# lmcinnes/pynndescent

Hardware: AMD Instinct MI355X
Metric: index build: points indexed/sec (recall@10 vs brute force reported alongside) (higher is better)
Workload: dtype f32

## Files before the change

include/pynnd_amd.h:

```cpp
#ifndef PYNND_AMD_H
#define PYNND_AMD_H

#include <stdint.h>

#ifdef __cplusplus
extern "C" {
#endif

#define NND_METRIC_SQEUCLIDEAN 0
#define NND_METRIC_ALT_COSINE 1

#define NND_ABI_VERSION 6

typedef struct nnd_handle_s *nnd_handle_t;

typedef struct nnd_params {
    int64_t n;
    int32_t dim;
    int32_t metric;
    int32_t n_neighbors;
    int32_t n_trees;
    int32_t leaf_size;
    int32_t max_depth;
    int32_t max_candidates;
// ... 11 lines not shown
#define NND_FLAG_NO_PREP 2
#define NND_FLAG_TEST_SELECT_WAVE 4
#define NND_FLAG_TEST_SMALL_REGIONS 8
#define NND_FLAG_TEST_ROUTE_PLAIN 16
#define NND_FLAG_TEST_FOREST_BY_TREE 32
#define NND_FLAG_TEST_FAIL 64
#define NND_FLAG_TEST_VANISH 128
#define NND_FLAG_TEST_SAMPLE_ATOMIC 256
#define NND_FLAG_TEST_FOREST_FALLBACK_TOPS 512
#define NND_FLAG_TEST_FOREST_FALLBACK_SHARE 1024
#define NND_TEST_FALLBACK_AT(flags) ((((flags) & 512) ? 1 : 0) + (((flags) & 1024) ? 2 : 0))
#define NND_FLAG_TEST_SAMPLE_NOMEM 2048
#define NND_FLAG_TEST_SELECT_HALF 4096
#define NND_FLAG_TEST_GATHER_INLINE 8192
#define NND_FLAG_TEST_JOIN_UNSTAGED 16384

typedef struct nnd_stats {
    int64_t n_iters_run;
    int64_t n_leaves;
    int64_t tree_levels;
    int64_t leaf_pairs;
    int64_t leaf_rows;
    int64_t join_pairs[64];
    int64_t join_rows[64];
    int64_t join_active[64];
    int64_t proposals[64];
    int64_t updates[64];
    float ms_prep, ms_forest, ms_leaf_init, ms_random_init, ms_descent, ms_finalize;
    float ms_sample[64], ms_join[64], ms_merge[64];
    int64_t join_mfma[64];
// ... 168 lines not shown
```

pynndescent_amd/_capi.py:

```python
import ctypes as C
import os

import numpy as np

_HERE = os.path.dirname(os.path.abspath(__file__))
LIB_PATH = os.environ.get("PYNND_AMD_LIB", os.path.join(_HERE, "libpynnd_amd.so"))

NND_METRIC_SQEUCLIDEAN = 0
NND_METRIC_ALT_COSINE = 1
METRIC_CODES = {"euclidean": NND_METRIC_SQEUCLIDEAN, "l2": NND_METRIC_SQEUCLIDEAN, "sqeuclidean": NND_METRIC_SQEUCLIDEAN,
                "cosine": NND_METRIC_ALT_COSINE}
NND_FLAG_NO_GRAPH = 1
NND_FLAG_NO_PREP = 2
NND_FLAG_TEST_SELECT_WAVE = 4
NND_FLAG_TEST_SMALL_REGIONS = 8
NND_FLAG_TEST_ROUTE_PLAIN = 16
NND_FLAG_TEST_FOREST_BY_TREE = 32
NND_FLAG_TEST_FAIL = 64
NND_FLAG_TEST_VANISH = 128
NND_FLAG_TEST_FOREST_FALLBACK_TOPS = 512
NND_FLAG_TEST_FOREST_FALLBACK_SHARE = 1024
NND_FLAG_TEST_GATHER_INLINE = 8192
NND_FLAG_TEST_JOIN_UNSTAGED = 16384
NND_FLAG_TEST_SELECT_HALF = 4096
NND_FLAG_TEST_SAMPLE_NOMEM = 2048
NND_FLAG_TEST_SAMPLE_ATOMIC = 256


class NNDParams(C.Structure):
    _fields_ = [
        ("n", C.c_int64),
        ("dim", C.c_int32),
        ("metric", C.c_int32),
        ("n_neighbors", C.c_int32),
        ("n_trees", C.c_int32),
        ("leaf_size", C.c_int32),
        ("max_depth", C.c_int32),
        ("max_candidates", C.c_int32),
        ("n_iters", C.c_int32),
        ("delta", C.c_float),
        ("rng_state", C.c_int64 * 3),
# ... 574 lines not shown
```

pynndescent_amd/csrc/capi.hip:

```cpp
#include <stdlib.h>
#include <string.h>

#include <atomic>
#include <mutex>
#include <string>
#include <thread>
#include <vector>

#include "common.h"
#include "state.h"

static thread_local char g_err[512] = {0};

static void gerr(const char *fmt, ...) {
    va_list ap;
    va_start(ap, fmt);
    vsnprintf(g_err, sizeof(g_err), fmt, ap);
    va_end(ap);
}

extern "C" int32_t nnd_abi_version(void) { return NND_ABI_VERSION; }
extern "C" const char *nnd_last_global_error(void) { return g_err; }
extern "C" const char *nnd_last_error(nnd_handle_t h) { return h ? h->err : g_err; }

// ... 49 lines not shown
#endif
    return m;
}

static void free_all(nnd_ctx *ctx) {
    auto F = [](void *p) {
        if (p) (void)hipFree(p);
    };
    if (ctx->x_owned) F((void *)ctx->x_orig);
    for (void *&a : ctx->slim_alloc) { F(a); a = nullptr; }
    F(ctx->xp); F(ctx->nrm); F(ctx->nr2); F(ctx->xh); F(ctx->mean); F(ctx->knn_e); F(ctx->knn_d); F(ctx->th); F(ctx->pbuf_r);
    F(ctx->pdirty); F(ctx->out_idx); F(ctx->out_dist);
    F(ctx->rv_pos); F(ctx->rv_in_cursor); F(ctx->rv_in_rec); F(ctx->rv_ov);
    for (int i = 0; i < 2; i++) { F(ctx->perm[i]); F(ctx->pos_seg[i]); F(ctx->seg_start[i]); F(ctx->seg_len[i]); }
    F(ctx->inv); F(ctx->side); F(ctx->side_pt); F(ctx->leaf_flag); F(ctx->scan_out); F(ctx->scan_blk); F(ctx->seg_nleft); F(ctx->seg_child);
    F(ctx->xs); F(ctx->xsh); F(ctx->nr2s); F(ctx->node_hf); F(ctx->node_hh); F(ctx->node_child); F(ctx->node_pack); F(ctx->node_hfc); F(ctx->route_roots); F(ctx->route_ws); F(ctx->s_leaf_depth);
    F(ctx->cell_count); F(ctx->cell_start); F(ctx->cell_depth); F(ctx->small_list);
    F(ctx->hyper); F(ctx->hyper_h); F(ctx->leaf_start); F(ctx->leaf_len); F(ctx->wl_start); F(ctx->wl_len); F(ctx->colsum_partial); F(ctx->counters_sum);
    if (ctx->h_pin) { (void)hipHostFree(ctx->h_pin); ctx->h_pin = nullptr; }
    if (ctx->h_tree_begin) { (void)hipHostFree(ctx->h_tree_begin); ctx->h_tree_begin = nullptr; }
    F(ctx->tree_begin_dev); F(ctx->counters);
    if (ctx->ev0) (void)hipEventDestroy(ctx->ev0);
    if (ctx->ev1) (void)hipEventDestroy(ctx->ev1);
    if (ctx->ev_spin) (void)hipEventDestroy(ctx->ev_spin);
    for (hipEvent_t e : ctx->tev) if (e) (void)hipEventDestroy(e);
    ctx->tev.clear();
    F(ctx->shard_bounds); F(ctx->shard_cursors);
    nnd_hub_tree_free(ctx);
    nnd_search_graph_free(ctx);
    if (ctx->stream && ctx->stream_owned) (void)hipStreamDestroy(ctx->stream);
}
// ... 147 lines not shown
                if (ctx->cell_leaf < 8) ctx->cell_leaf = 8;
                const int64_t Ps = (int64_t)p->n_trees * ctx->s_m;
                ctx->node_cap = Ps / (ctx->cell_leaf / 4 > 1 ? ctx->cell_leaf / 4 : 1) + 4 * p->n_trees + 64;
                ctx->cell_cap = ctx->node_cap + p->n_trees;
                ctx->max_segs += ctx->cell_cap;
                if ((rc = dalloc(ctx, &ctx->xs, (size_t)ctx->s_m * ctx->dp))) break;
                if ((rc = dalloc(ctx, &ctx->xsh, (size_t)ctx->s_m * ctx->dp))) break;
                if ((rc = dalloc(ctx, &ctx->nr2s, (size_t)ctx->s_m))) break;
                if ((rc = dalloc(ctx, &ctx->node_hf, (size_t)ctx->node_cap * (ctx->dp + 4)))) break;
                if ((rc = dalloc(ctx, &ctx->node_hh, (size_t)ctx->node_cap * ctx->dp))) break;
                if ((rc = dalloc(ctx, &ctx->node_child, (size_t)ctx->node_cap * 2))) break;
                if ((rc = dalloc(ctx, &ctx->node_pack, (size_t)ctx->node_cap * (2 * ctx->dp + 16)))) break;
                if ((rc = dalloc(ctx, &ctx->node_hfc, (size_t)ctx->node_cap * (ctx->dp + 4)))) break;
                if ((rc = dalloc(ctx, &ctx->route_roots, (size_t)4096))) break;
                if ((rc = dalloc(ctx, &ctx->s_leaf_depth, (size_t)Ps))) break;
                if ((rc = dalloc(ctx, &ctx->cell_count, (size_t)ctx->cell_cap))) break;
                if ((rc = dalloc(ctx, &ctx->cell_start, (size_t)ctx->cell_cap))) break;
                if ((rc = dalloc(ctx, &ctx->cell_depth, (size_t)ctx->cell_cap))) break;
                if ((rc = dalloc(ctx, &ctx->small_list, (size_t)ctx->cell_cap * 3))) break;
            }
            const size_t S = (size_t)ctx->max_segs;
            for (int i = 0; i < 2 && !rc; i++) {
                if ((rc = dalloc(ctx, &ctx->perm[i], P))) break;
                if ((rc = dalloc(ctx, &ctx->pos_seg[i], P))) break;
                if ((rc = dalloc(ctx, &ctx->seg_start[i], S))) break;
                if ((rc = dalloc(ctx, &ctx->seg_len[i], S))) break;
            }
            if (rc) break;
            if ((rc = dalloc(ctx, &ctx->inv, P))) break;
            if ((rc = dalloc(ctx, &ctx->side, P))) break;
// ... 833 lines not shown
```

pynndescent_amd/csrc/rpforest.hip:

```cpp
#include <atomic>
#include <chrono>

#include "common.h"
#include "state.h"

#define RP_EPS 1e-8f

static constexpr int SCAN_ITEMS = 8;
static constexpr int SCAN_BLOCK = 256;
static constexpr int SCAN_TILE = SCAN_ITEMS * SCAN_BLOCK;

__global__ void k_forest_init(int32_t *__restrict__ perm, int32_t *__restrict__ pos_seg, uint8_t *__restrict__ leaf_flag,
                              int32_t *__restrict__ inv, int64_t n, int64_t P, int splittable) {
    int64_t g = (int64_t)blockIdx.x * blockDim.x + threadIdx.x;
    if (g >= P) return;
    int64_t t = g / n;
    int64_t i = g - t * n;
    perm[g] = (int32_t)i;
    inv[g] = splittable ? (int32_t)t : -1;
    pos_seg[g] = splittable ? (int32_t)t : -1;
    leaf_flag[g] = (!splittable && i == 0) ? 1 : 0;
}
__global__ void k_forest_init_segs(int32_t *__restrict__ seg_start, int32_t *__restrict__ seg_len, int n_trees,
                                   int64_t n) {
    int t = blockIdx.x * blockDim.x + threadIdx.x;
    if (t < n_trees) {
        seg_start[t] = (int32_t)(t * n);
        seg_len[t] = (int32_t)n;
    }
}

__global__ __launch_bounds__(256) void k_hyperplane(const float *__restrict__ xp, int dp, const int32_t *__restrict__ perm,
                                                    const int32_t *__restrict__ seg_start,
                                                    const int32_t *__restrict__ seg_len, int n_segs, int angular,
                                                    uint32_t seed, int depth, float *__restrict__ hyper, int hs,
                                                    uint16_t *__restrict__ hyper_h, uint32_t pos_bias, const float *__restrict__ scal) {
    int lane = nnd_lane();
    int s = blockIdx.x * (blockDim.x >> 6) + (threadIdx.x >> 6);
    if (s >= n_segs) return;
    int a = seg_start[s], len = seg_len[s];
    uint32_t li = nnd_hash3(seed, (uint32_t)a + pos_bias, (uint32_t)(2 * depth)) % (uint32_t)len;
    uint32_t ri = nnd_hash3(seed, (uint32_t)a + pos_bias, (uint32_t)(2 * depth + 1)) % (uint32_t)len;
    if (ri == li) ri = (ri + 1) % (uint32_t)len;
    const float *xl = xp + (int64_t)perm[a + li] * dp;
    const float *xr = xp + (int64_t)perm[a + ri] * dp;
    float *h = hyper + (int64_t)s * hs;
    uint16_t *hb = hyper_h + (int64_t)s * dp;
    const float hsc = scal[0], hinv = 1.0f / hsc;
    float acc = 0.0f, sq = 0.0f, res = 0.0f;
    for (int j = lane; j < dp; j += 64) {
        float l = xl[j], r = xr[j];
        float v = l - r;
        h[j] = v;
        if (!angular) {
            const uint16_t b = nnd_f32_to_h16(v, hsc);
            hb[j] = b;
            const float e = v - nnd_h16_to_f32(b, hinv);
            res += e * e;
        }
        acc += angular ? v * v : v * (l + r);
        sq += v * v;
    }
// ... 14 lines not shown
        if (lane == 0) {
            h[dp] = 0.0f;
            h[dp + 1] = nh * inv;
            h[dp + 2] = sqrtf(res) * 1.000001f;
        }
    } else {
        res = nnd_wave_sum_f32(res);
        if (lane == 0) {
            h[dp] = -0.5f * acc;
            h[dp + 1] = sqrtf(sq);
            h[dp + 2] = sqrtf(res) * 1.000001f;
        }
    }
}

#define RP_BAND 0.00786f
#define RP_ACC 3e-5f
#ifdef NND_RP_ALWAYS_EXACT
#define RP_IN_BAND(m, band) ((band) >= 0.0f || (m) == (m))
#else
#define RP_IN_BAND(m, band) (!(fabsf(m) > (band)))
#endif
__device__ __forceinline__ float rp_band(float xnorm, float rx, float hnorm, float rh) {
    return rx * hnorm + (xnorm + rx) * rh + RP_ACC * hnorm * xnorm + RP_EPS;
}
__device__ __forceinline__ uint32_t rp_bf16_up(float v) { return (__float_as_uint(v) + 0xFFFFu) >> 16; }
typedef _Float16 rp_h16x2 __attribute__((ext_vector_type(2)));
__device__ __forceinline__ float rp_dot8(uint4 q, uint4 p, float acc) {
    acc = __builtin_amdgcn_fdot2(__builtin_bit_cast(rp_h16x2, q.x), __builtin_bit_cast(rp_h16x2, p.x), acc, false);
    acc = __builtin_amdgcn_fdot2(__builtin_bit_cast(rp_h16x2, q.y), __builtin_bit_cast(rp_h16x2, p.y), acc, false);
// ... 15 lines not shown
        acc += a.x * b.x + a.y * b.y + a.z * b.z + a.w * b.w;
    }
    return rp_quad_sum(acc);
}
__device__ __forceinline__ uint8_t rp_side(float m, float band, const float *__restrict__ xf_row, const float *h, float off,
                                           int dp, int sub, uint32_t seed, uint32_t key, int depth) {
#ifdef NND_RP_NORECHECK
    if (band < 0.0f) m = rp_exact_quad(xf_row, h, dp, sub) + off;
#else
    if (RP_IN_BAND(m, band)) m = rp_exact_quad(xf_row, h, dp, sub) + off;
#endif
    if (fabsf(m) < RP_EPS) return (uint8_t)(nnd_hash3(seed ^ 0x5bd1e995u, key, (uint32_t)depth) & 1u);
    return m > 0.0f ? 0 : 1;
}

__global__ __launch_bounds__(256) void k_margin(const float *__restrict__ xp, const uint16_t *__restrict__ xh,
                                                const float2 *__restrict__ nr, int metric, int dp,
                                                const int32_t *__restrict__ perm, const int32_t *__restrict__ pos_seg,
                                                int64_t P, const float *__restrict__ hyper, int hs,
                                                const uint16_t *__restrict__ hyper_h, uint32_t seed, int depth,
                                                uint8_t *__restrict__ side, uint32_t pos_bias, const float *__restrict__ scal) {
    const int sub = threadIdx.x & 3;
    const int64_t g = (int64_t)blockIdx.x * (blockDim.x >> 2) + (threadIdx.x >> 2);
    const int s = g < P ? pos_seg[g] : -1;
    if (s < 0) return;
    const int64_t pt = perm[g];
    const uint4 *x8 = (const uint4 *)(xh + pt * dp);
    const uint4 *h8 = (const uint4 *)(hyper_h + (int64_t)s * dp);
    const float *h = hyper + (int64_t)s * hs;
    const float2 nrv = nr[pt];
    const float xn = nrv.x, rx = nrv.y, off = h[dp], hnorm = h[dp + 1], rh = h[dp + 2];
    float acc = 0.0f;
    for (int c = sub; c < (dp >> 3); c += 16) {
        uint4 q[4], p[4];
#pragma unroll
        for (int j = 0; j < 4; j++) {
            const int cc = c + 4 * j < (dp >> 3) ? c + 4 * j : c;
            q[j] = x8[cc];
            p[j] = h8[cc];
        }
#pragma unroll
        for (int j = 0; j < 4; j++)
            if (c + 4 * j < (dp >> 3)) acc = rp_dot8(q[j], p[j], acc);
    }
    const float m = rp_quad_sum(acc) * scal[1] + off;
    const float band = rp_band(metric == 0 ? sqrtf(xn) : xn, rx, hnorm, rh);
    const uint8_t sd = rp_side(m, band, xp + pt * dp, h, off, dp, sub, seed, (uint32_t)g + pos_bias, depth);
    if (sub == 0) side[g] = sd;
}

__global__ __launch_bounds__(256) void k_margin_fused(const float *__restrict__ xp, const uint16_t *__restrict__ xh,
                                                      const float2 *__restrict__ nr, int metric, int dp, int64_t n,
                                                      int n_trees, const int32_t *__restrict__ seg_pt,
                                                      const float *__restrict__ hyper, int hs,
                                                      const uint16_t *__restrict__ hyper_h, uint32_t seed, int depth,
                                                      uint8_t *__restrict__ side_pt, uint32_t pos_bias, const float *__restrict__ scal) {
    const int sub = threadIdx.x & 3;
    const int64_t i = (int64_t)blockIdx.x * (blockDim.x >> 2) + (threadIdx.x >> 2);
    if (i >= n) return;
    const uint4 *x8 = (const uint4 *)(xh + i * dp);
    const float2 nrv = nr[i];
    const float xn = nrv.x, rx = nrv.y;
    const float xnorm = metric == 0 ? sqrtf(xn) : xn;
    const int nch = dp >> 3;
    for (int t0 = 0; t0 < n_trees; t0 += 4) {
        int sg[4];
        float acc[4];
#pragma unroll
        for (int u = 0; u < 4; u++) {
            sg[u] = t0 + u < n_trees ? seg_pt[(int64_t)(t0 + u) * n + i] : -1;
            acc[u] = 0.0f;
        }
        if (sg[0] < 0 && sg[1] < 0 && sg[2] < 0 && sg[3] < 0) continue;
// ... 12 lines not shown
                    if (c + 4 * j < nch) acc[u] = rp_dot8(q[j], p[j], acc[u]);
            }
        }
#pragma unroll
        for (int u = 0; u < 4; u++) {
            if (sg[u] < 0) continue;
            const float *h = hyper + (int64_t)sg[u] * hs;
            const float off = h[dp], hnorm = h[dp + 1], rh = h[dp + 2];
            const float m = rp_quad_sum(acc[u]) * scal[1] + off;
            const float band = rp_band(xnorm, rx, hnorm, rh);
            const int64_t slot = (int64_t)(t0 + u) * n + i;
            const uint8_t sd = rp_side(m, band, xp + i * dp, h, off, dp, sub, seed, (uint32_t)slot + pos_bias, depth);
            if (sub == 0) side_pt[slot] = sd;
        }
    }
}

__device__ __forceinline__ int scan_flag(int mode, const int32_t *pos_seg, const uint8_t *bytes, int64_t g, int64_t P) {
    if (g >= P) return 0;
    if (mode == 0) {
        const int sg = pos_seg[g];
        const uint8_t b = bytes[g];
        return (sg >= 0) & (b == 0);
    }
    return bytes[g] ? 1 : 0;
}

__global__ __launch_bounds__(SCAN_BLOCK) void k_scan_reduce(int mode, const int32_t *__restrict__ pos_seg,
                                                            uint8_t *__restrict__ bytes, int64_t P,
                                                            int32_t *__restrict__ blk, const int32_t *__restrict__ perm,
// ... 243 lines not shown
    }
    if (active_pos) atomicAdd((unsigned long long *)&counters[CNT_LEAVES], (unsigned long long)active_pos);
    if (max_stay) atomicMax((unsigned long long *)&counters[CNT_SCRATCH + 3], (unsigned long long)max_stay);
    if (host_words) {
        __syncthreads();
        if (threadIdx.x == 0) {
#pragma unroll
            for (int q = 0; q < 6; q++)
                host_words[q] = __hip_atomic_load(&counters[CNT_ACTIVE_SEGS + q], __ATOMIC_RELAXED, __HIP_MEMORY_SCOPE_AGENT);
            __threadfence_system();
            __hip_atomic_store(&host_words[6], seq, __ATOMIC_RELEASE, __HIP_MEMORY_SCOPE_SYSTEM);
        }
    }
}

__global__ void k_scatter(const int32_t *__restrict__ perm, const int32_t *__restrict__ pos_seg,
                          const uint8_t *__restrict__ side, const int32_t *__restrict__ scan,
                          const int32_t *__restrict__ seg_start, const int32_t *__restrict__ nleft,
                          const int32_t *__restrict__ seg_child, int64_t P, int64_t n, int32_t *__restrict__ perm_out,
                          int32_t *__restrict__ pos_seg_out, int32_t *__restrict__ inv) {
    int64_t g = (int64_t)blockIdx.x * blockDim.x + threadIdx.x;
    if (g >= P) return;
    int s = pos_seg[g];
    if (s < 0) {
        perm_out[g] = perm[g];
        pos_seg_out[g] = -1;
        return;
    }
    int a = seg_start[s];
    int nl = nleft[s];
    int right;
    int64_t dest;
    if (nl < 0) {
        nl = -nl - 1;
        int off = (int)(g - a);
        right = off & 1;
        dest = right ? (int64_t)a + nl + (off >> 1) : (int64_t)a + (off >> 1);
    } else {
        int L = scan[g] - scan[a];
        right = side[g];
        dest = right ? (int64_t)a + nl + ((int)(g - a) - L) : (int64_t)a + L;
    }
    int32_t p = perm[g];
    perm_out[dest] = p;
    pos_seg_out[dest] = seg_child[2 * s + right];
    if (inv) inv[(g / n) * n + p] = seg_child[2 * s + right];
}

#ifndef NND_FIN_MAX
#define NND_FIN_MAX 2048
#endif
static constexpr int FIN_MAX = NND_FIN_MAX;
#ifndef NND_BIG_MAX
#define NND_BIG_MAX 8192
#endif
static constexpr int BIG_MAX = NND_BIG_MAX;
static constexpr int FIN_STACK = 40;
static constexpr int FIN_SMALL = 512;
static constexpr int FIN_WS = 40;

__device__ __forceinline__ void rp_top2_push(uint64_t &a, uint64_t &b, uint64_t k) {
// ... 1086 lines not shown
    const long long nfin = ctx->h_pin[34];
    if (nfin > ctx->max_segs) {
        ctx->set_error("rp-forest: %lld finisher segments exceed the allocation of %lld", nfin, (long long)ctx->max_segs);
        return 1;
    }
    if (nfin > 0) {
        hipLaunchKernelGGL((k_finish_subtrees<false, 256, FIN_MAX>), dim3((unsigned)nfin), dim3(256), fin_smem_bytes(dp, FIN_MAX),
                           ctx->stream, FIN_ARGS(fin_start, fin_len, fin_depth, 0, nfin), (int32_t *)nullptr, (uint8_t *)nullptr,
                           FIN_MAX, fin_start, fin_len, fin_depth, fin_count, tm, ctx->mean + ctx->dp);
        NND_HIP_CHECK(hipGetLastError());
    }
#undef FIN_ARGS
    return 0;
}

static int forest_levels(nnd_ctx *ctx, forest_view &v) {
    const int64_t n = v.n, P = v.P;
    const int T = v.T > 0 ? v.T : ctx->p.n_trees, dp = ctx->dp, leaf_size = v.leaf_size, max_depth = ctx->p.max_depth;
    const uint32_t pos_bias = (uint32_t)((int64_t)v.tree_bias * n);
    rp_tree_map tm;
    tm.tree_bias = v.tree_bias;
    const int angular = ctx->p.metric == NND_METRIC_ALT_COSINE;
    const int hs = dp + 4;
    int32_t *scan_total = (int32_t *)(ctx->counters + CNT_SCRATCH);
    int splittable = (n > leaf_size && max_depth > 0) ? 1 : 0;
    int cur = 0;
    unsigned gridP = (unsigned)((P + 255) / 256);
    hipLaunchKernelGGL(k_forest_init, dim3(gridP), dim3(256), 0, ctx->stream, ctx->perm[0], ctx->pos_seg[0],
                       ctx->leaf_flag, ctx->inv, n, P, splittable);
    hipLaunchKernelGGL(k_forest_init_segs, dim3((T + 63) / 64), dim3(64), 0, ctx->stream, ctx->seg_start[0],
// ... 8 lines not shown
    int32_t *fin_depth = fin_len + ctx->max_segs;
    int64_t node_base = 0;
    long long *flag_words = (ctx->h_pin_dev && !ctx->wait_hook && !nnd_knob("NND_NO_LEVEL_FLAG")) ? ctx->h_pin_dev + 40 : nullptr;
    NND_HIP_CHECK(hipMemsetAsync(ctx->counters + CNT_SCRATCH + 1, 0, sizeof(long long), ctx->stream));
    if (!v.record && S > 0 && n <= fin_max) {
        std::vector<int32_t> h_s(T), h_l(T), h_d(T, 0);
        for (int t = 0; t < T; t++) { h_s[t] = (int32_t)(t * n); h_l[t] = (int32_t)n; }
        NND_HIP_CHECK(hipMemcpyAsync(fin_start, h_s.data(), sizeof(int32_t) * T, hipMemcpyHostToDevice, ctx->stream));
        NND_HIP_CHECK(hipMemcpyAsync(fin_len, h_l.data(), sizeof(int32_t) * T, hipMemcpyHostToDevice, ctx->stream));
        NND_HIP_CHECK(hipMemcpyAsync(fin_depth, h_d.data(), sizeof(int32_t) * T, hipMemcpyHostToDevice, ctx->stream));
        long long cntf = T;
        NND_HIP_CHECK(hipMemcpyAsync(ctx->counters + CNT_SCRATCH + 1, &cntf, sizeof(long long), hipMemcpyHostToDevice, ctx->stream));
        NND_HIP_CHECK(hipStreamSynchronize(ctx->stream));
        S = 0;
    }
    while (S > 0) {
        if (S > ctx->max_segs) {
            ctx->set_error("rp-forest: %lld segments exceed the allocation of %lld", (long long)S, (long long)ctx->max_segs);
            return 1;
        }
        if (v.record && node_base + S > ctx->node_cap) {
            if (nnd_knob("NND_FOREST_DEBUG")) fprintf(stderr, "forest: fallback at line %d\n", __LINE__);
            return 2;
        }
        if (v.record) v.level_base.push_back(node_base);
        float *hyper = v.record ? ctx->node_hf + node_base * hs : ctx->hyper;
        uint16_t *hyper_h = v.record ? ctx->node_hh + node_base * dp : ctx->hyper_h;
        hipLaunchKernelGGL(k_hyperplane, dim3((unsigned)((S + 3) / 4)), dim3(256), 0, ctx->stream, v.xp, dp,
                           ctx->perm[cur], ctx->seg_start[cur], ctx->seg_len[cur], (int)S, angular, ctx->tree_seed, depth,
                           hyper, hs, hyper_h, pos_bias, ctx->mean + ctx->dp);
// ... 48 lines not shown
        if (!v.record && S > 0 && (active_pos * 2 < 3 * n) && next[5] <= BIG_MAX) {
            if (launch_finishers(ctx, ctx->perm[cur], ctx->perm[1 - cur], ctx->seg_start[cur], ctx->seg_len[cur], nullptr, depth, S, 0, tm)) return 1;
            v.cur = cur;
            v.depth = depth;
            v.n_nodes = node_base;
            return 0;
        }
    }
    v.cur = cur;
    v.depth = depth;
    v.n_nodes = node_base;
    if (v.record) {
        v.level_base.push_back(node_base);
        NND_HIP_CHECK(hipMemcpyAsync(ctx->h_pin + 34, ctx->counters + CNT_SCRATCH + 1, sizeof(long long), hipMemcpyDeviceToHost, ctx->stream));
        NND_HIP_CHECK(nnd_sync_spin(ctx));
        const long long nfin = ctx->h_pin[34];
        if (nfin > ctx->max_segs || node_base + nfin + 1 >= ctx->node_cap) {
            if (nnd_knob("NND_FOREST_DEBUG")) fprintf(stderr, "forest: fallback at line %d\n", __LINE__);
            return 2;
        }
        v.n_low = node_base;
        v.high_lo = ctx->node_cap;
        if (nfin > 0) {
            int *flags = (int *)(ctx->counters + CNT_SCRATCH + 2);
            NND_HIP_CHECK(hipMemsetAsync(flags, 0, 2 * sizeof(int), ctx->stream));
            rp_record rec{ctx->node_hf, ctx->node_hh, ctx->node_child, ctx->s_leaf_depth, hs, (int)ctx->node_cap - 1,
                          (int)(ctx->node_cap - 1 - nfin), (int)node_base, flags, flags + 1, 0, FIN_MAX};
            rp_record rs = rec, rl = rec;
            rs.min_len = 0; rs.max_len = FIN_SMALL;
            rl.min_len = FIN_SMALL + 1; rl.max_len = FIN_MAX;
// ... 569 lines not shown
```

pynndescent_amd/csrc/state.h:

```cpp
#pragma once
#include <mutex>
#include <hip/hip_runtime.h>
#include <stdarg.h>
#include <stdint.h>
#include <stdio.h>

#include <vector>

#include "../../include/pynnd_amd.h"

#include <stdlib.h>
static inline const char *nnd_knob(const char *name) {
#ifdef NND_EXPERIMENT_KNOBS
    return getenv(name);
#else
    (void)name;
    return nullptr;
#endif
}

enum {
    CNT_ACCEPT = 0,
    CNT_PAIRS,
    CNT_ROWS,
// ... 83 lines not shown
    int cell_leaf = 0;
    int early_stop = 8;
    float *xs = nullptr;
    uint16_t *xsh = nullptr;
    float2 *nr2s = nullptr;
    int64_t node_cap = 0, cell_cap = 0;
    float *node_hf = nullptr;
    uint16_t *node_hh = nullptr;
    int32_t *node_child = nullptr;
    unsigned char *node_pack = nullptr;
    float *node_hfc = nullptr;
    int32_t *route_roots = nullptr;
    unsigned char *route_ws = nullptr;
    size_t route_ws_cap = 0;
    int32_t *s_leaf_depth = nullptr;
    int32_t *cell_count = nullptr, *cell_start = nullptr, *cell_depth = nullptr;
    int32_t *small_list = nullptr;
    int32_t *leaf_start = nullptr, *leaf_len = nullptr;
    double *colsum_partial = nullptr;
    size_t colsum_cap = 0;
    int64_t leaf_cap = 0;
    std::vector<int32_t> h_leaf_start, h_leaf_len;
    bool h_leaf_valid = false;
    long long *tree_begin_dev = nullptr;
    long long *h_tree_begin = nullptr;
    int32_t *wl_start = nullptr, *wl_len = nullptr;
    int64_t wl_cap = 0;
    int64_t n_leaves = 0;
    int32_t max_leaf = 0;
    std::vector<int64_t> tree_leaf_begin;
// ... 153 lines not shown
```

Baseline: 51.86 million.

## Drive RP-forest level passes from device state with host lookahead launches

Adds a device-driven level loop for the random-projection forest build. Each level's hyperplane, margin, scan, children and scatter kernels read the segment count from a device workspace. This lets the host enqueue several levels ahead without a blocking sync to learn each level's segment count. The device publishes counts through a pinned host ring, and the host spins on it only when the lookahead window is full. This removes per-level host round-trips but adds grid-stride kernels sized for a worst-case bound, ticket-based scan ordering, and more complex error and fallback handling.

After: 51.92 million, median of 6. Within noise of the previous version (+0.1%).

```diff
diff --git a/include/pynnd_amd.h b/include/pynnd_amd.h
--- a/include/pynnd_amd.h
+++ b/include/pynnd_amd.h
@@ -49,6 +49,7 @@
 #define NND_FLAG_TEST_SELECT_HALF 4096
 #define NND_FLAG_TEST_GATHER_INLINE 8192
 #define NND_FLAG_TEST_JOIN_UNSTAGED 16384
+#define NND_FLAG_TEST_FOREST_LEVELS_HOST 32768
 
 typedef struct nnd_stats {
     int64_t n_iters_run;
diff --git a/pynndescent_amd/_capi.py b/pynndescent_amd/_capi.py
--- a/pynndescent_amd/_capi.py
+++ b/pynndescent_amd/_capi.py
@@ -25,6 +25,7 @@
 NND_FLAG_TEST_SELECT_HALF = 4096
 NND_FLAG_TEST_SAMPLE_NOMEM = 2048
 NND_FLAG_TEST_SAMPLE_ATOMIC = 256
+NND_FLAG_TEST_FOREST_LEVELS_HOST = 32768
 
 
 class NNDParams(C.Structure):
diff --git a/pynndescent_amd/csrc/capi.hip b/pynndescent_amd/csrc/capi.hip
--- a/pynndescent_amd/csrc/capi.hip
+++ b/pynndescent_amd/csrc/capi.hip
@@ -87,7 +87,7 @@
     F(ctx->rv_pos); F(ctx->rv_in_cursor); F(ctx->rv_in_rec); F(ctx->rv_ov);
     for (int i = 0; i < 2; i++) { F(ctx->perm[i]); F(ctx->pos_seg[i]); F(ctx->seg_start[i]); F(ctx->seg_len[i]); }
     F(ctx->inv); F(ctx->side); F(ctx->side_pt); F(ctx->leaf_flag); F(ctx->scan_out); F(ctx->scan_blk); F(ctx->seg_nleft); F(ctx->seg_child);
-    F(ctx->xs); F(ctx->xsh); F(ctx->nr2s); F(ctx->node_hf); F(ctx->node_hh); F(ctx->node_child); F(ctx->node_pack); F(ctx->node_hfc); F(ctx->route_roots); F(ctx->route_ws); F(ctx->s_leaf_depth);
+    F(ctx->xs); F(ctx->xsh); F(ctx->nr2s); F(ctx->node_hf); F(ctx->node_hh); F(ctx->node_child); F(ctx->node_pack); F(ctx->node_hfc); F(ctx->route_roots); F(ctx->route_ws); F(ctx->s_leaf_depth); F(ctx->lvl_ws);
     F(ctx->cell_count); F(ctx->cell_start); F(ctx->cell_depth); F(ctx->small_list);
     F(ctx->hyper); F(ctx->hyper_h); F(ctx->leaf_start); F(ctx->leaf_len); F(ctx->wl_start); F(ctx->wl_len); F(ctx->colsum_partial); F(ctx->counters_sum);
     if (ctx->h_pin) { (void)hipHostFree(ctx->h_pin); ctx->h_pin = nullptr; }
@@ -265,6 +265,7 @@
                 if ((rc = dalloc(ctx, &ctx->node_hfc, (size_t)ctx->node_cap * (ctx->dp + 4)))) break;
                 if ((rc = dalloc(ctx, &ctx->route_roots, (size_t)4096))) break;
                 if ((rc = dalloc(ctx, &ctx->s_leaf_depth, (size_t)Ps))) break;
+                if ((rc = dalloc(ctx, &ctx->lvl_ws, (size_t)(32 + Ps / 2048 + 2)))) break;
                 if ((rc = dalloc(ctx, &ctx->cell_count, (size_t)ctx->cell_cap))) break;
                 if ((rc = dalloc(ctx, &ctx->cell_start, (size_t)ctx->cell_cap))) break;
                 if ((rc = dalloc(ctx, &ctx->cell_depth, (size_t)ctx->cell_cap))) break;
diff --git a/pynndescent_amd/csrc/rpforest.hip b/pynndescent_amd/csrc/rpforest.hip
--- a/pynndescent_amd/csrc/rpforest.hip
+++ b/pynndescent_amd/csrc/rpforest.hip
@@ -30,22 +30,14 @@
     }
 }
 
-__global__ __launch_bounds__(256) void k_hyperplane(const float *__restrict__ xp, int dp, const int32_t *__restrict__ perm,
-                                                    const int32_t *__restrict__ seg_start,
-                                                    const int32_t *__restrict__ seg_len, int n_segs, int angular,
-                                                    uint32_t seed, int depth, float *__restrict__ hyper, int hs,
-                                                    uint16_t *__restrict__ hyper_h, uint32_t pos_bias, const float *__restrict__ scal) {
-    int lane = nnd_lane();
-    int s = blockIdx.x * (blockDim.x >> 6) + (threadIdx.x >> 6);
-    if (s >= n_segs) return;
-    int a = seg_start[s], len = seg_len[s];
+__device__ __forceinline__ void rp_hyperplane_wave(const float *xp, int dp, const int32_t *perm, int a, int len, int angular,
+                                                   uint32_t seed, int depth, float *h, uint16_t *hb, uint32_t pos_bias,
+                                                   const float *scal, int lane) {
     uint32_t li = nnd_hash3(seed, (uint32_t)a + pos_bias, (uint32_t)(2 * depth)) % (uint32_t)len;
     uint32_t ri = nnd_hash3(seed, (uint32_t)a + pos_bias, (uint32_t)(2 * depth + 1)) % (uint32_t)len;
     if (ri == li) ri = (ri + 1) % (uint32_t)len;
     const float *xl = xp + (int64_t)perm[a + li] * dp;
     const float *xr = xp + (int64_t)perm[a + ri] * dp;
-    float *h = hyper + (int64_t)s * hs;
-    uint16_t *hb = hyper_h + (int64_t)s * dp;
     const float hsc = scal[0], hinv = 1.0f / hsc;
     float acc = 0.0f, sq = 0.0f, res = 0.0f;
     for (int j = lane; j < dp; j += 64) {
@@ -90,6 +82,17 @@
     }
 }
 
+__global__ __launch_bounds__(256) void k_hyperplane(const float *__restrict__ xp, int dp, const int32_t *__restrict__ perm,
+                                                    const int32_t *__restrict__ seg_start,
+                                                    const int32_t *__restrict__ seg_len, int n_segs, int angular,
+                                                    uint32_t seed, int depth, float *__restrict__ hyper, int hs,
+                                                    uint16_t *__restrict__ hyper_h, uint32_t pos_bias, const float *__restrict__ scal) {
+    int s = blockIdx.x * (blockDim.x >> 6) + (threadIdx.x >> 6);
+    if (s >= n_segs) return;
+    rp_hyperplane_wave(xp, dp, perm, seg_start[s], seg_len[s], angular, seed, depth, hyper + (int64_t)s * hs, hyper_h + (int64_t)s * dp,
+                       pos_bias, scal, nnd_lane());
+}
+
 #define RP_BAND 0.00786f
 #define RP_ACC 3e-5f
 #ifdef NND_RP_ALWAYS_EXACT
@@ -135,14 +138,10 @@
     return m > 0.0f ? 0 : 1;
 }
 
-__global__ __launch_bounds__(256) void k_margin(const float *__restrict__ xp, const uint16_t *__restrict__ xh,
-                                                const float2 *__restrict__ nr, int metric, int dp,
-                                                const int32_t *__restrict__ perm, const int32_t *__restrict__ pos_seg,
-                                                int64_t P, const float *__restrict__ hyper, int hs,
-                                                const uint16_t *__restrict__ hyper_h, uint32_t seed, int depth,
-                                                uint8_t *__restrict__ side, uint32_t pos_bias, const float *__restrict__ scal) {
-    const int sub = threadIdx.x & 3;
-    const int64_t g = (int64_t)blockIdx.x * (blockDim.x >> 2) + (threadIdx.x >> 2);
+__device__ __forceinline__ void rp_margin_pos(int64_t g, int sub, const float *xp, const uint16_t *xh, const float2 *nr, int metric,
+                                              int dp, const int32_t *perm, const int32_t *pos_seg, int64_t P, const float *hyper,
+                                              int hs, const uint16_t *hyper_h, uint32_t seed, int depth, uint8_t *side,
+                                              uint32_t pos_bias, const float *scal) {
     const int s = g < P ? pos_seg[g] : -1;
     if (s < 0) return;
     const int64_t pt = perm[g];
@@ -169,15 +168,20 @@
     const uint8_t sd = rp_side(m, band, xp + pt * dp, h, off, dp, sub, seed, (uint32_t)g + pos_bias, depth);
     if (sub == 0) side[g] = sd;
 }
-
-__global__ __launch_bounds__(256) void k_margin_fused(const float *__restrict__ xp, const uint16_t *__restrict__ xh,
-                                                      const float2 *__restrict__ nr, int metric, int dp, int64_t n,
-                                                      int n_trees, const int32_t *__restrict__ seg_pt,
-                                                      const float *__restrict__ hyper, int hs,
-                                                      const uint16_t *__restrict__ hyper_h, uint32_t seed, int depth,
-                                                      uint8_t *__restrict__ side_pt, uint32_t pos_bias, const float *__restrict__ scal) {
-    const int sub = threadIdx.x & 3;
-    const int64_t i = (int64_t)blockIdx.x * (blockDim.x >> 2) + (threadIdx.x >> 2);
+__global__ __launch_bounds__(256) void k_margin(const float *__restrict__ xp, const uint16_t *__restrict__ xh,
+                                                const float2 *__restrict__ nr, int metric, int dp,
+                                                const int32_t *__restrict__ perm, const int32_t *__restrict__ pos_seg,
+                                                int64_t P, const float *__restrict__ hyper, int hs,
+                                                const uint16_t *__restrict__ hyper_h, uint32_t seed, int depth,
+                                                uint8_t *__restrict__ side, uint32_t pos_bias, const float *__restrict__ scal) {
+    const int64_t g = (int64_t)blockIdx.x * (blockDim.x >> 2) + (threadIdx.x >> 2);
+    rp_margin_pos(g, threadIdx.x & 3, xp, xh, nr, metric, dp, perm, pos_seg, P, hyper, hs, hyper_h, seed, depth, side, pos_bias, scal);
+}
+
+__device__ __forceinline__ void rp_margin_point(int64_t i, int sub, const float *xp, const uint16_t *xh, const float2 *nr, int metric,
+                                                int dp, int64_t n, int n_trees, const int32_t *seg_pt, const float *hyper, int hs,
+                                                const uint16_t *hyper_h, uint32_t seed, int depth, uint8_t *side_pt,
+                                                uint32_t pos_bias, const float *scal) {
     if (i >= n) return;
     const uint4 *x8 = (const uint4 *)(xh + i * dp);
     const float2 nrv = nr[i];
@@ -220,6 +224,15 @@
             if (sub == 0) side_pt[slot] = sd;
         }
     }
+}
+__global__ __launch_bounds__(256) void k_margin_fused(const float *__restrict__ xp, const uint16_t *__restrict__ xh,
+                                                      const float2 *__restrict__ nr, int metric, int dp, int64_t n,
+                                                      int n_trees, const int32_t *__restrict__ seg_pt,
+                                                      const float *__restrict__ hyper, int hs,
+                                                      const uint16_t *__restrict__ hyper_h, uint32_t seed, int depth,
+                                                      uint8_t *__restrict__ side_pt, uint32_t pos_bias, const float *__restrict__ scal) {
+    const int64_t i = (int64_t)blockIdx.x * (blockDim.x >> 2) + (threadIdx.x >> 2);
+    rp_margin_point(i, threadIdx.x & 3, xp, xh, nr, metric, dp, n, n_trees, seg_pt, hyper, hs, hyper_h, seed, depth, side_pt, pos_bias, scal);
 }
 
 __device__ __forceinline__ int scan_flag(int mode, const int32_t *pos_seg, const uint8_t *bytes, int64_t g, int64_t P) {
@@ -493,13 +506,10 @@
     }
 }
 
-__global__ void k_scatter(const int32_t *__restrict__ perm, const int32_t *__restrict__ pos_seg,
-                          const uint8_t *__restrict__ side, const int32_t *__restrict__ scan,
-                          const int32_t *__restrict__ seg_start, const int32_t *__restrict__ nleft,
-                          const int32_t *__restrict__ seg_child, int64_t P, int64_t n, int32_t *__restrict__ perm_out,
-                          int32_t *__restrict__ pos_seg_out, int32_t *__restrict__ inv) {
-    int64_t g = (int64_t)blockIdx.x * blockDim.x + threadIdx.x;
-    if (g >= P) return;
+__device__ __forceinline__ void rp_scatter_pos(int64_t g, const int32_t *perm, const int32_t *pos_seg, const uint8_t *side,
+                                               const int32_t *scan, const int32_t *seg_start, const int32_t *nleft,
+                                               const int32_t *seg_child, int64_t n, int32_t *perm_out, int32_t *pos_seg_out,
+                                               int32_t *inv) {
     int s = pos_seg[g];
     if (s < 0) {
         perm_out[g] = perm[g];
@@ -524,6 +534,299 @@
     perm_out[dest] = p;
     pos_seg_out[dest] = seg_child[2 * s + right];
     if (inv) inv[(g / n) * n + p] = seg_child[2 * s + right];
+}
+__global__ void k_scatter(const int32_t *__restrict__ perm, const int32_t *__restrict__ pos_seg,
+                          const uint8_t *__restrict__ side, const int32_t *__restrict__ scan,
+                          const int32_t *__restrict__ seg_start, const int32_t *__restrict__ nleft,
+                          const int32_t *__restrict__ seg_child, int64_t P, int64_t n, int32_t *__restrict__ perm_out,
+                          int32_t *__restrict__ pos_seg_out, int32_t *__restrict__ inv) {
+    int64_t g = (int64_t)blockIdx.x * blockDim.x + threadIdx.x;
+    if (g >= P) return;
+    rp_scatter_pos(g, perm, pos_seg, side, scan, seg_start, nleft, seg_child, n, perm_out, pos_seg_out, inv);
+}
+
+enum {
+    RP_LVL_STATE = 0,
+    RP_LVL_TK_SCAN = 16, RP_LVL_ERR,
+    RP_LVL_TILES = 32
+};
+#define RP_RLX(p) __hip_atomic_load((p), __ATOMIC_RELAXED, __HIP_MEMORY_SCOPE_AGENT)
+__device__ __forceinline__ int rp_ticket(unsigned long long *ctr, int d, unsigned long long *err) {
+    __shared__ int tk;
+    if (threadIdx.x == 0) {
+        const long long t = (long long)(__hip_atomic_fetch_add(ctr, 1ull, __ATOMIC_RELAXED, __HIP_MEMORY_SCOPE_AGENT) -
+                                        (unsigned long long)d * gridDim.x);
+        tk = t >= 0 && t < (long long)gridDim.x ? (int)t : -1;
+        if (tk < 0) __hip_atomic_store(err, 1ull, __ATOMIC_RELAXED, __HIP_MEMORY_SCOPE_AGENT);
+    }
+    __syncthreads();
+    return tk;
+}
+__device__ __forceinline__ bool rp_lvl_fused(const unsigned long long *st, int64_t n, int dp) {
+    const long long S = (long long)st[0], active = (long long)st[1];
+    return st[3] != 0 && S * (long long)dp * 2 <= ((long long)6 << 20) && active * 2 >= 3 * n;
+}
+
+__global__ void k_lvl_init(unsigned long long *ws, int n_words, long long S0, long long P) {
+    for (int i = blockIdx.x * blockDim.x + threadIdx.x; i < n_words; i += gridDim.x * blockDim.x) ws[i] = 0;
+    if (blockIdx.x == 0 && threadIdx.x == 0) {
+        ws[RP_LVL_STATE + 0] = (unsigned long long)S0;
+        ws[RP_LVL_STATE + 1] = (unsigned long long)P;
+        ws[RP_LVL_STATE + 3] = 1;
+    }
+}
+
+__global__ __launch_bounds__(256) void k_lvl_hyper(const unsigned long long *ws, int d, const float *xp, int dp, const int32_t *perm,
+                                                   const int32_t *seg_start, const int32_t *seg_len, int32_t *nleft, int angular,
+                                                   uint32_t seed, float *node_hf, uint16_t *node_hh, int hs, uint32_t pos_bias,
+                                                   const float *scal) {
+    const unsigned long long *st = ws + RP_LVL_STATE + 8 * (d & 1);
+    const long long S = (long long)st[0];
+    if (S <= 0) return;
+    const int64_t node_base = (int64_t)st[2];
+    float *hyper = node_hf + node_base * hs;
+    uint16_t *hyper_h = node_hh + node_base * dp;
+    for (long long s = (long long)blockIdx.x * 4 + (threadIdx.x >> 6); s < S; s += (long long)gridDim.x * 4) {
+        rp_hyperplane_wave(xp, dp, perm, seg_start[s], seg_len[s], angular, seed, d, hyper + s * hs, hyper_h + s * dp, pos_bias, scal,
+                           nnd_lane());
+        if (nnd_lane() == 0) nleft[s] = 0;
+    }
+}
+
+__global__ __launch_bounds__(256) void k_lvl_margin(const unsigned long long *ws, int d, const float *xp, const uint16_t *xh,
+                                                    const float2 *nr, int metric, int dp, int64_t n, int T, int64_t P,
+                                                    const int32_t *perm, const int32_t *pos_seg, const int32_t *inv, uint32_t seed,
+                                                    const float *node_hf, const uint16_t *node_hh, int hs, uint8_t *side,
+                                                    uint8_t *side_pt, uint32_t pos_bias, const float *scal) {
+    const unsigned long long *st = ws + RP_LVL_STATE + 8 * (d & 1);
+    if ((long long)st[0] <= 0) return;
+    const int64_t node_base = (int64_t)st[2];
+    const float *hyper = node_hf + node_base * hs;
+    const uint16_t *hyper_h = node_hh + node_base * dp;
+    const int64_t q0 = (int64_t)blockIdx.x * 64 + (threadIdx.x >> 2), qs = (int64_t)gridDim.x * 64;
+    const int sub = threadIdx.x & 3;
+    if (rp_lvl_fused(st, n, dp)) {
+        for (int64_t i = q0; i < n; i += qs)
+            rp_margin_point(i, sub, xp, xh, nr, metric, dp, n, T, inv, hyper, hs, hyper_h, seed, d, side_pt, pos_bias, scal);
+    } else {
+        for (int64_t g = q0; g < P; g += qs)
+            rp_margin_pos(g, sub, xp, xh, nr, metric, dp, perm, pos_seg, P, hyper, hs, hyper_h, seed, d, side, pos_bias, scal);
+    }
+}
+
+__global__ __launch_bounds__(SCAN_BLOCK) void k_lvl_scan(unsigned long long *ws, int d, int64_t n, int64_t P, int dp,
+                                                         const int32_t *pos_seg, const int32_t *perm, const uint8_t *side_pt,
+                                                         uint8_t *side, int32_t *scan_out, int32_t *nleft) {
+    const unsigned long long *st = ws + RP_LVL_STATE + 8 * (d & 1);
+    if ((long long)st[0] <= 0) return;
+    const bool fused = rp_lvl_fused(st, n, dp);
+    const int tile = rp_ticket(ws + RP_LVL_TK_SCAN, d, ws + RP_LVL_ERR);
+    if (tile < 0) return;
+    const int lane = nnd_lane(), w = threadIdx.x >> 6;
+    const int64_t base = (int64_t)tile * SCAN_TILE + (int64_t)threadIdx.x * SCAN_ITEMS;
+    int sg[SCAN_ITEMS], f[SCAN_ITEMS];
+    int s = 0;
+    if (fused) {
+        const int64_t tb0 = base < P ? (base / n) * n : 0;
+        int pt[SCAN_ITEMS];
+#pragma unroll
+        for (int i = 0; i < SCAN_ITEMS; i++) {
+            const int64_t g = base + i < P ? base + i : P - 1;
+            sg[i] = pos_seg[g];
+            pt[i] = perm[g];
+        }
+#pragma unroll
+        for (int i = 0; i < SCAN_ITEMS; i++) {
+            const int64_t g = base + i;
+            int64_t tb = tb0;
+            while (g >= tb + n && tb + n < P) tb += n;
+            const uint8_t sd = side_pt[tb + pt[i]];
+            if (g >= P) sg[i] = -1;
+            f[i] = sg[i] >= 0 && sd == 0;
+            if (sg[i] >= 0) side[g] = sd;
+        }
+    } else {
+#pragma unroll
+        for (int i = 0; i < SCAN_ITEMS; i++) {
+            const int64_t g = base + i;
+            sg[i] = g < P ? pos_seg[g] : -1;
+            const uint8_t b = g < P ? side[g] : 1;
+            f[i] = (sg[i] >= 0) & (b == 0);
+        }
+    }
+#pragma unroll
+    for (int i = 0; i < SCAN_ITEMS; i++) s += f[i];
+    const int sg_prev = base > 0 && base - 1 < P ? pos_seg[base - 1] : -2;
+    const int sg_next = base + SCAN_ITEMS < P ? pos_seg[base + SCAN_ITEMS] : -2;
+    __shared__ int wsum[SCAN_BLOCK / 64];
+    __shared__ int tile_prefix;
+    const int incl = nnd_wave_incl_scan_i32(s);
+    if (lane == 63) wsum[w] = incl;
+    __syncthreads();
+    int woff = 0, agg = 0;
+#pragma unroll
+    for (int i = 0; i < SCAN_BLOCK / 64; i++) {
+        woff += i < w ? wsum[i] : 0;
+        agg += wsum[i];
+    }
+    if (w == 0) {
+        unsigned long long *fl = ws + RP_LVL_TILES;
+        const unsigned tagA = 2u * (unsigned)d + 1u, tagI = tagA + 1u;
+        int prefix = 0;
+        if (tile > 0) {
+            if (lane == 0) __hip_atomic_store(&fl[tile], ((unsigned long long)tagA << 32) | (unsigned)agg, __ATOMIC_RELAXED, __HIP_MEMORY_SCOPE_AGENT);
+            unsigned spins = 0;
+            for (int64_t j0 = tile - 1; j0 >= 0;) {
+                const int64_t j = j0 - lane;
+                const unsigned long long v = j >= 0 ? RP_RLX(&fl[j]) : ((unsigned long long)tagI << 32);
+                const unsigned tag = (unsigned)(v >> 32);
+                const unsigned long long incl_mask = __ballot(tag == tagI), wait_mask = __ballot(tag < tagA);
+                const int fi = incl_mask ? __builtin_ctzll(incl_mask) : 64;
+                const unsigned long long need = fi >= 63 ? ~0ull : ((1ull << (fi + 1)) - 1);
+                if (wait_mask & need) {
+                    if (++spins > (1u << 22)) {
+                        if (lane == 0) __hip_atomic_store(ws + RP_LVL_ERR, 1ull, __ATOMIC_RELAXED, __HIP_MEMORY_SCOPE_AGENT);
+                        break;
+                    }
+                    __builtin_amdgcn_s_sleep(1);
+                    continue;
+                }
+                prefix += nnd_wave_sum_i32(lane <= fi && j >= 0 ? (int)(unsigned)v : 0);
+                if (fi < 64) break;
+                j0 -= 64;
+            }
+        }
+        if (lane == 0) {
+            __hip_atomic_store(&fl[tile], ((unsigned long long)tagI << 32) | (unsigned)(prefix + agg), __ATOMIC_RELAXED, __HIP_MEMORY_SCOPE_AGENT);
+            tile_prefix = prefix;
+        }
+    }
+    __syncthreads();
+    int run = tile_prefix + woff + incl - s;
+#pragma unroll
+    for (int i = 0; i < SCAN_ITEMS; i++) {
+        const int64_t g = base + i;
+        if (g < P) scan_out[g] = run;
+        if (sg[i] >= 0) {
+            const int prev = i > 0 ? sg[i - 1] : sg_prev, next = i + 1 < SCAN_ITEMS ? sg[i + 1] : sg_next;
+            if (prev != sg[i]) atomicAdd(&nleft[sg[i]], -run);
+            if (next != sg[i]) atomicAdd(&nleft[sg[i]], run + f[i]);
+        }
+        run += f[i];
+    }
+}
+
+__global__ __launch_bounds__(256) void k_lvl_children(
+    unsigned long long *ws, int d, int64_t n, int64_t P, int dp, int max_depth, int leaf_size, int fin_max, int early_stop,
+    int64_t max_segs, int64_t node_cap, const int32_t *seg_start, const int32_t *seg_len, int32_t *nleft, int32_t *seg_child,
+    int32_t *next_start, int32_t *next_len, int32_t *fin_start, int32_t *fin_len, int32_t *fin_depth, long long *fin_count,
+    int32_t *node_child, int32_t *leaf_depth, uint8_t *leaf_flag, long long *host_ring, long long *host_seq, long long seq_base) {
+    unsigned long long *st = ws + RP_LVL_STATE + 8 * (d & 1);
+    const long long S = (long long)st[0];
+    if (S <= 0) {
+        if (threadIdx.x == 0) ws[RP_LVL_STATE + 8 * ((d + 1) & 1)] = 0;
+        return;
+    }
+    const bool fused = rp_lvl_fused(st, n, dp);
+    const int node_base = (int)st[2];
+    const long long active = (long long)st[1];
+    int child_can_split = (max_depth - (d + 1)) > 0 ? 1 : 0;
+    if (early_stop > 0 && active * early_stop < P) child_can_split = 0;
+    __shared__ int part[256], partf[256];
+    __shared__ unsigned long long active_sum;
+    __shared__ int ovf, s_next;
+    const int ns = (int)S;
+    const int chunk = (ns + 255) / 256;
+    const int s0 = threadIdx.x * chunk, s1 = s0 + chunk < ns ? s0 + chunk : ns;
+    int cnt = 0, cntf = 0;
+    for (int s = s0; s < s1; s++) {
+        const int len = seg_len[s];
+        int nl = nleft[s];
+        if (nl == 0 || nl == len) {
+            nl = (len + 1) / 2;
+            nleft[s] = -nl - 1;
+        }
+        const int lens[2] = {nl, len - nl};
+#pragma unroll
+        for (int c = 0; c < 2; c++)
+            if (child_can_split && lens[c] > leaf_size) {
+                if (lens[c] > fin_max) cnt++; else cntf++;
+            }
+    }
+    part[threadIdx.x] = cnt;
+    partf[threadIdx.x] = cntf;
+    __syncthreads();
+    if (threadIdx.x == 0) {
+        int run = 0, runf = (int)*fin_count;
+        for (int i = 0; i < 256; i++) {
+            int v = part[i]; part[i] = run; run += v;
+            int vf = partf[i]; partf[i] = runf; runf += vf;
+        }
+        ovf = (run > max_segs || (int64_t)node_base + S + run > node_cap || runf > max_segs || RP_RLX(ws + RP_LVL_ERR) != 0) ? 1 : 0;
+        if (!ovf) *fin_count = runf;
+        s_next = ovf ? 0 : run;
+        active_sum = 0;
+    }
+    __syncthreads();
+    long long active_pos = 0;
+    if (!ovf) {
+        int run = part[threadIdx.x], runf = partf[threadIdx.x];
+        for (int s = s0; s < s1; s++) {
+            const int a = seg_start[s], len = seg_len[s];
+            int nl = nleft[s];
+            if (nl < 0) nl = -nl - 1;
+            const int lens[2] = {nl, len - nl};
+            const int starts[2] = {a, a + nl};
+#pragma unroll
+            for (int c = 0; c < 2; c++) {
+                if (child_can_split && lens[c] > leaf_size) {
+                    if (lens[c] > fin_max) {
+                        next_start[run] = starts[c];
+                        next_len[run] = lens[c];
+                        node_child[2 * (node_base + s) + c] = node_base + ns + run;
+                        seg_child[2 * s + c] = run++;
+                        active_pos += lens[c];
+                    } else {
+                        fin_start[runf] = starts[c];
+                        fin_len[runf] = lens[c];
+                        fin_depth[runf] = d + 1;
+                        node_child[2 * (node_base + s) + c] = (int)node_cap - 1 - runf;
+                        runf++;
+                        seg_child[2 * s + c] = -1;
+                    }
+                } else {
+                    seg_child[2 * s + c] = -1;
+                    if (lens[c] > 0) leaf_flag[starts[c]] = 1;
+                    node_child[2 * (node_base + s) + c] = -2 - starts[c];
+                    if (lens[c] > 0) leaf_depth[starts[c]] = d + 1;
+                }
+            }
+        }
+    }
+    if (active_pos) atomicAdd(&active_sum, (unsigned long long)active_pos);
+    __syncthreads();
+    if (threadIdx.x == 0) {
+        unsigned long long *nx = ws + RP_LVL_STATE + 8 * ((d + 1) & 1);
+        const long long S_next = s_next;
+        nx[0] = (unsigned long long)S_next;
+        nx[1] = active_sum;
+        nx[2] = (unsigned long long)(node_base + S);
+        nx[3] = fused ? 1 : 0;
+        host_ring[d & 15] = ovf ? -1 : S_next;
+        __threadfence_system();
+        __hip_atomic_store(host_seq, seq_base + d + 1, __ATOMIC_RELEASE, __HIP_MEMORY_SCOPE_SYSTEM);
+    }
+}
+
+__global__ __launch_bounds__(256) void k_lvl_scatter(const unsigned long long *ws, int d, int64_t n, int64_t P, int dp,
+                                                     const int32_t *perm, const int32_t *pos_seg, const uint8_t *side,
+                                                     const int32_t *scan, const int32_t *seg_start, const int32_t *nleft,
+                                                     const int32_t *seg_child, int32_t *perm_out, int32_t *pos_seg_out, int32_t *inv) {
+    const unsigned long long *st = ws + RP_LVL_STATE + 8 * (d & 1);
+    if ((long long)st[0] <= 0 || ws[RP_LVL_ERR] != 0) return;
+    int32_t *inv_w = rp_lvl_fused(st, n, dp) ? inv : nullptr;
+    for (int64_t g = (int64_t)blockIdx.x * blockDim.x + threadIdx.x; g < P; g += (int64_t)gridDim.x * blockDim.x)
+        rp_scatter_pos(g, perm, pos_seg, side, scan, seg_start, nleft, seg_child, n, perm_out, pos_seg_out, inv_w);
 }
 
 #ifndef NND_FIN_MAX
@@ -1640,6 +1943,86 @@
     return 0;
 }
 
+static constexpr int RP_LVL_AHEAD = 4;
+static int forest_levels_device(nnd_ctx *ctx, forest_view &v, int64_t S0, int *cur_out, int *depth_out, int64_t *node_base_out) {
+    const int64_t n = v.n, P = v.P;
+    const int T = v.T > 0 ? v.T : ctx->p.n_trees, dp = ctx->dp, hs = dp + 4, max_depth = ctx->p.max_depth;
+    const int angular = ctx->p.metric == NND_METRIC_ALT_COSINE;
+    const uint32_t pos_bias = (uint32_t)((int64_t)v.tree_bias * n);
+    const int n_tiles = (int)((P + SCAN_TILE - 1) / SCAN_TILE);
+    const int n_words = RP_LVL_TILES + n_tiles;
+    if (S0 > ctx->max_segs) {
+        ctx->set_error("rp-forest: %lld segments exceed the allocation of %lld", (long long)S0, (long long)ctx->max_segs);
+        return 1;
+    }
+    if (S0 > ctx->node_cap) return 2;
+    const int64_t s_bound = std::max<int64_t>(T, P / (v.fin_max + 1));
+    const int H = (int)std::min<int64_t>(std::max<int64_t>((s_bound + 3) / 4, 1), 1024);
+    const int g_margin = (int)std::min<int64_t>(std::max<int64_t>((P + 63) / 64, 1), 8192);
+    const int g_scat = (int)std::min<int64_t>(std::max<int64_t>((P + 255) / 256, 1), 4096);
+    int32_t *fin_start = ctx->seg_child + 2 * ctx->max_segs;
+    int32_t *fin_len = fin_start + ctx->max_segs;
+    int32_t *fin_depth = fin_len + ctx->max_segs;
+    unsigned long long *ws = ctx->lvl_ws;
+    hipLaunchKernelGGL(k_lvl_init, dim3(1), dim3(256), 0, ctx->stream, ws, n_words, (long long)S0, (long long)P);
+    const long long seq0 = ctx->flag_seq;
+    const volatile long long *ring = ctx->h_pin + 16, *seqw = ctx->h_pin + 47;
+    std::vector<long long> Sk{(long long)S0};
+    int e = 0;
+    while (Sk.back() > 0) {
+        const int known = (int)Sk.size() - 1;
+        if (e - known < RP_LVL_AHEAD) {
+            const int c = e & 1;
+            hipLaunchKernelGGL(k_lvl_hyper, dim3((unsigned)H), dim3(256), 0, ctx->stream, ws, e, v.xp, dp, ctx->perm[c], ctx->seg_start[c],
+                               ctx->seg_len[c], ctx->seg_nleft, angular, ctx->tree_seed, ctx->node_hf, ctx->node_hh, hs, pos_bias, ctx->mean + dp);
+            hipLaunchKernelGGL(k_lvl_margin, dim3((unsigned)g_margin), dim3(256), 0, ctx->stream, ws, e, v.xp, v.xh, v.nr, ctx->p.metric, dp,
+                               n, T, P, ctx->perm[c], ctx->pos_seg[c], ctx->inv, ctx->tree_seed, ctx->node_hf, ctx->node_hh, hs, ctx->side,
+                               ctx->side_pt, pos_bias, ctx->mean + dp);
+            hipLaunchKernelGGL(k_lvl_scan, dim3((unsigned)n_tiles), dim3(SCAN_BLOCK), 0, ctx->stream, ws, e, n, P, dp, ctx->pos_seg[c],
+                               ctx->perm[c], ctx->side_pt, ctx->side, ctx->scan_out, ctx->seg_nleft);
+            hipLaunchKernelGGL(k_lvl_children, dim3(1), dim3(256), 0, ctx->stream, ws, e, n, P, dp, max_depth, v.leaf_size, v.fin_max,
+                               ctx->early_stop, (int64_t)ctx->max_segs, (int64_t)ctx->node_cap, ctx->seg_start[c], ctx->seg_len[c],
+                               ctx->seg_nleft, ctx->seg_child, ctx->seg_start[1 - c], ctx->seg_len[1 - c], fin_start, fin_len, fin_depth,
+                               ctx->counters + CNT_SCRATCH + 1, ctx->node_child, ctx->s_leaf_depth, ctx->leaf_flag, ctx->h_pin_dev + 16,
+                               ctx->h_pin_dev + 47, seq0);
+            hipLaunchKernelGGL(k_lvl_scatter, dim3((unsigned)g_scat), dim3(256), 0, ctx->stream, ws, e, n, P, dp, ctx->perm[c], ctx->pos_seg[c],
+                               ctx->side, ctx->scan_out, ctx->seg_start[c], ctx->seg_nleft, ctx->seg_child, ctx->perm[1 - c],
+                               ctx->pos_seg[1 - c], ctx->inv);
+            NND_HIP_CHECK(hipGetLastError());
+            e++;
+            continue;
+        }
+        const auto t_spin = std::chrono::steady_clock::now();
+        unsigned spins = 0;
+        while (*seqw < seq0 + known + 1) {
+            if ((++spins & 0xFFFFu) == 0 && std::chrono::steady_clock::now() - t_spin > std::chrono::seconds(30)) {
+                ctx->flag_seq = seq0 + e;
+                ctx->set_error("rp-forest: the device did not hand over the segment count of level %d within 30 s", known);
+                return 1;
+            }
+        }
+        std::atomic_thread_fence(std::memory_order_acquire);
+        Sk.push_back((long long)ring[known & 15]);
+    }
+    ctx->flag_seq = seq0 + e;
+    NND_HIP_CHECK(hipMemcpyAsync(ctx->h_pin + 33, ws + RP_LVL_ERR, sizeof(long long), hipMemcpyDeviceToHost, ctx->stream));
+    if (Sk.back() < 0) {
+        if (nnd_knob("NND_FOREST_DEBUG")) fprintf(stderr, "forest: fallback at line %d\n", __LINE__);
+        NND_HIP_CHECK(nnd_sync_spin(ctx));
+        return 2;
+    }
+    const int depth = (int)Sk.size() - 1;
+    int64_t node_base = 0;
+    for (int d = 0; d < depth; d++) {
+        v.level_base.push_back(node_base);
+        node_base += Sk[d];
+    }
+    *cur_out = depth & 1;
+    *depth_out = depth;
+    *node_base_out = node_base;
+    return 0;
+}
+
 static int forest_levels(nnd_ctx *ctx, forest_view &v) {
     const int64_t n = v.n, P = v.P;
     const int T = v.T > 0 ? v.T : ctx->p.n_trees, dp = ctx->dp, leaf_size = v.leaf_size, max_depth = ctx->p.max_depth;
@@ -1678,6 +2061,14 @@
         NND_HIP_CHECK(hipStreamSynchronize(ctx->stream));
         S = 0;
     }
+    const bool dev_levels = v.record && flag_words && ctx->lvl_ws && !(ctx->p.flags & NND_FLAG_TEST_FOREST_LEVELS_HOST);
+    bool dev_ran = false;
+    if (dev_levels && S > 0) {
+        const int rc = forest_levels_device(ctx, v, S, &cur, &depth, &node_base);
+        if (rc) return rc;
+        S = 0;
+        dev_ran = true;
+    }
     while (S > 0) {
         if (S > ctx->max_segs) {
             ctx->set_error("rp-forest: %lld segments exceed the allocation of %lld", (long long)S, (long long)ctx->max_segs);
@@ -1756,6 +2147,10 @@
         v.level_base.push_back(node_base);
         NND_HIP_CHECK(hipMemcpyAsync(ctx->h_pin + 34, ctx->counters + CNT_SCRATCH + 1, sizeof(long long), hipMemcpyDeviceToHost, ctx->stream));
         NND_HIP_CHECK(nnd_sync_spin(ctx));
+        if (dev_ran && ctx->h_pin[33] != 0) {
+            ctx->set_error("rp-forest: a wait of the device-driven level passes timed out");
+            return 1;
+        }
         const long long nfin = ctx->h_pin[34];
         if (nfin > ctx->max_segs || node_base + nfin + 1 >= ctx->node_cap) {
             if (nnd_knob("NND_FOREST_DEBUG")) fprintf(stderr, "forest: fallback at line %d\n", __LINE__);
diff --git a/pynndescent_amd/csrc/state.h b/pynndescent_amd/csrc/state.h
--- a/pynndescent_amd/csrc/state.h
+++ b/pynndescent_amd/csrc/state.h
@@ -121,6 +121,7 @@
     unsigned char *route_ws = nullptr;
     size_t route_ws_cap = 0;
     int32_t *s_leaf_depth = nullptr;
+    unsigned long long *lvl_ws = nullptr;
     int32_t *cell_count = nullptr, *cell_start = nullptr, *cell_depth = nullptr;
     int32_t *small_list = nullptr;
     int32_t *leaf_start = nullptr, *leaf_len = nullptr;
```
